# wonjune-kang/llm-speech-summarization

Hardware: AMD Instinct MI355X
Metric: generated tokens/s of end-to-end generate_audio_response steps (encode + prefill + 256-token greedy decode), HuBERT-large -> Llama-3.2-3B; audio-sec/s reported beside it, encoder stage alone and in the pipeline (higher is better)
Workload: dtype bf16

## Files before the change

### llm-speech-summarization_amd/csrc/api.hip

```cpp
#include <stdarg.h>
#include <stdlib.h>

#include <atomic>
#include <mutex>

#include "common.h"

static thread_local char g_err[512] = "";

void sl_set_error(const char* fmt, ...) {
  va_list ap;
  va_start(ap, fmt);
  vsnprintf(g_err, sizeof(g_err), fmt, ap);
  va_end(ap);
}

extern "C" const char* sl_last_error(void) { return g_err; }

extern "C" int sl_version(void) { return SL_ABI_VERSION; }

extern "C" int sl_device_arch(char* buf, int n) {
  SL_CHECK_ARG(buf != nullptr && n > 0, "sl_device_arch: bad buffer");
  int dev = 0;
  SL_HIP(hipGetDevice(&dev));
// ... 35 lines not shown
  e.stream_min_m = env_int("SL_STREAM_MIN_M", 26);
  if (e.stream_min_m < 16) e.stream_min_m = 26;
  e.disable_t256 = getenv("SL_DISABLE_T256") != nullptr;
  e.t256_min_tiles = env_int("SL_T256_MIN_TILES", 512);
  e.t256_min_k = env_int("SL_T256_MIN_K", 1024);
  e.t256_phased = env_int("SL_T256_PHASED", 1);
  e.t256_by_rounds_pad = env_int("SL_T256_BY_ROUNDS_PAD", 1);
  e.decode_tiled = env_int("SL_DECODE_TILED", 1);
  e.stream_k = env_int("SL_STREAM_K", 1);
  e.split_k = env_int("SL_SPLIT_K", 1);
  e.wgrad_tr = env_int("SL_WGRAD_TR", 1);
  e.tt_max_splits = env_int("SL_TT_MAX_SPLITS", 8);
  e.lnbwd_nw = env_int("SL_LNBWD_NW", 16);
  e.skinny_alt = env_int("SL_SKINNY_ALT", 0);
  e.prefill_share_prefix = env_int("SL_PREFILL_SHARE_PREFIX", 1);
  e.gemm_ko = env_int("SL_GEMM_KO", 0);
  { const char* sp = getenv("SL_GEMM_STAMP_PTR"); e.gemm_stamp_ptr = (sp && sp[0]) ? strtoull(sp, nullptr, 16) : 0ull; }
  const char* g = getenv("SL_DISABLE_GLDS");
  e.disable_glds = (g && g[0] == '1') ? 1 : ((g && g[0] == '2') ? 2 : 0);
  e.direct_epilogue = env_int("SL_DIRECT_EPILOGUE", 0);
  e.gemm_gm = env_int("SL_GEMM_GM", 8);
  e.attn_full_min = env_int("SL_ATTN_FULL_MIN", 32);
  e.attn_force_split = getenv("SL_ATTN_FORCE_SPLIT") != nullptr;
  { const int ks = env_int("SL_ATTN_DECODE_KS", 128); e.attn_decode_ks = (ks == 64 || ks == 65) ? ks : 128; }
  e.attn_split_merge = env_int("SL_ATTN_SPLIT_MERGE", -1);
  e.attn_generic = env_int("SL_ATTN_GENERIC", 0);
  e.attn_qt = env_int("SL_ATTN_QT", 0);
  e.norm_single_row = env_int("SL_NORM_SINGLE_ROW", 0);
  e.no_ln_fold = env_int("SL_NO_LN_FOLD", 0);
  e.no_swap_epilogue = env_int("SL_NO_SWAP_EPILOGUE", 0);
// ... 47 lines not shown
```

### llm-speech-summarization_amd/csrc/common.h

```cpp
#pragma once
#include <hip/hip_runtime.h>
#include <stdint.h>
#include <stdio.h>
#include <string.h>

#include "../../include/speechllm.h"

void sl_set_error(const char* fmt, ...);

#define SL_CHECK_ARG(cond, ...)      \
  do {                               \
    if (!(cond)) {                   \
      sl_set_error(__VA_ARGS__);     \
      return SL_ERR_ARG;             \
    }                                \
  } while (0)

#define SL_CHECK_LAUNCH(what)                                                        \
  do {                                                                               \
    hipError_t e__ = hipGetLastError();                                              \
    if (e__ != hipSuccess) {                                                         \
      sl_set_error("%s: %s", what, hipGetErrorString(e__));                          \
      return SL_ERR_LAUNCH;                                                          \
    }                                                                                \
// ... 254 lines not shown
  int direct_epilogue;
  int gemm_gm;
  int attn_full_min;
  int attn_force_split;
  int attn_decode_ks;
  int attn_split_merge;
  int attn_generic;
  int attn_qt;
  int norm_single_row;
  int no_ln_fold;
  int no_wgrad_stream;
  int gemm_log;
  int no_swap_epilogue;
  int decode_tiled;
  int prefill_share_prefix;
  int skinny_alt;
  int tt_max_splits;
  int lnbwd_nw;
  int wgrad_tr;
  int split_k;
  int stream_k;
  int gemm_ko;
  unsigned long long gemm_stamp_ptr;
  int stream_splits, stream_nwv, stream_mt;
  int stream_wide;
  int stream_wsplits;
  int stream_fixup;
  int stream_nl;
};
const SlEnv& sl_env();
// ... 22 lines not shown
```

### llm-speech-summarization_amd/csrc/gemm_stream.hip

```cpp
#include <stdlib.h>

#include <atomic>

#include "gemm_internal.h"

struct StreamX {
  float* part;
  float* part_ss;
  int splits, sps;
  int np;
  int* cnt;
  float* ss_part;
};

__device__ __forceinline__ void st_sc1_16(float* ptr, const f32x4& v) {
  asm volatile("global_store_dwordx4 %0, %1, off sc1" ::"v"(ptr), "v"(v) : "memory");
}
__device__ __forceinline__ void ld_sc1_16(f32x4& v, const float* ptr) {
  asm volatile("global_load_dwordx4 %0, %1, off sc1" : "=v"(v) : "v"(ptr) : "memory");
}
__device__ __forceinline__ void vm_drain16(f32x4 (&v)[16]) {
  asm volatile("s_waitcnt vmcnt(0)"
               : "+v"(v[0]), "+v"(v[1]), "+v"(v[2]), "+v"(v[3]), "+v"(v[4]), "+v"(v[5]), "+v"(v[6]), "+v"(v[7]), "+v"(v[8]), "+v"(v[9]), "+v"(v[10]),
                 "+v"(v[11]), "+v"(v[12]), "+v"(v[13]), "+v"(v[14]), "+v"(v[15])
// ... 478 lines not shown
      if (old == nbv - 1) s.cnt[1024 + mblock] = 0;
    }
    __builtin_amdgcn_s_barrier();
    if (!fx_last[1]) return;
    if (tid < 256) {
      const int m = m0 + tid;
      if (m < p.M) {
        float t = 0.f;
        for (int j = 0; j < nbv; ++j) t += __hip_atomic_load(&s.ss_part[(int64_t)j * p.M + m], __ATOMIC_RELAXED, __HIP_MEMORY_SCOPE_AGENT);
        sx.rstd_out[m] = rsqrtf(t / (float)p.N + sx.eps);
      }
    }
  }
}

template <typename T, int ACT, bool ROWSTAT>
__global__ __launch_bounds__(ROWSTAT ? 1024 : 256) void gemm_stream_reduce_kernel(GemmP p, SkinnyX sx, StreamX s) {
  constexpr bool PAIRS = (ACT == SL_ACT_SILU_MUL || ACT == SL_ACT_ROPE_KV);
  static_assert(!ROWSTAT || ACT == SL_ACT_NONE, "row statistics ride on the plain (+residual) epilogue");
  const int nfrag = (p.N + 15) >> 4;
  const int nunits = PAIRS ? (nfrag + 1) / 2 : nfrag;
  int q, unit, m;
  if constexpr (ROWSTAT) {
    m = blockIdx.x; q = threadIdx.x & 3; unit = threadIdx.x >> 2;
  } else {
    const int64_t idx = (int64_t)blockIdx.x * 256 + threadIdx.x;
    q = (int)(idx & 3);
    unit = (int)((idx >> 2) % nunits);
    m = (int)(idx / (4 * (int64_t)nunits));
    if (m >= p.M) return;
  }
  const bool live = unit < nunits;
  const int gf = PAIRS ? 2 * unit : unit;
  f32x4 a4 = {0.f, 0.f, 0.f, 0.f}, b4 = {0.f, 0.f, 0.f, 0.f};
  float ssum = 0.f;
  const bool stats_here = sx.fuse_rms && !sx.rstd_in;
  if (live) {
    constexpr int UN = 8;
    for (int sp0 = 0; sp0 < s.splits; sp0 += UN) {
      f32x4 va[UN], vb[UN];
#pragma unroll
      for (int u = 0; u < UN; ++u) {
        const int sp = sp0 + u < s.splits ? sp0 + u : s.splits - 1;
        const float* row = s.part + ((int64_t)sp * p.M + m) * s.np + gf * 16 + 4 * q;
        va[u] = *(const f32x4*)row;
        if constexpr (PAIRS) vb[u] = *(const f32x4*)(row + 16);
      }
#pragma unroll
      for (int u = 0; u < UN; ++u) {
        if (sp0 + u < s.splits) {
          a4 += va[u];
          if constexpr (PAIRS) b4 += vb[u];
        }
      }
    }
    if (stats_here)
      for (int sp = 0; sp < s.splits; ++sp) ssum += s.part_ss[(int64_t)sp * p.M + m];
  }
  const float rs = sx.rstd_in ? sx.rstd_in[m] : (stats_here ? rsqrtf(ssum / (float)p.K + sx.eps) : 1.0f);
  float a[4], b[4];
#pragma unroll
  for (int i = 0; i < 4; ++i) { a[i] = a4[i] * rs; b[i] = b4[i] * rs; }
  if constexpr (ROWSTAT) {
    __shared__ float wsum[17];
    float sq = 0.f;
    float kept[4] = {0.f, 0.f, 0.f, 0.f};
    if (live) {
      const T* bias = (const T*)p.bias;
#pragma unroll
      for (int i = 0; i < 4; ++i) {
        const int col = gf * 16 + 4 * q + i;
        if (col >= p.N) continue;
        float v = a[i];
        if (bias) v += to_f32(bias[col]);
        if (p.res) v += p.res_f32 ? ((const float*)p.res)[(int64_t)m * p.ldr + col] : to_f32(((const T*)p.res)[(int64_t)m * p.ldr + col]);
        if (p.out_f32) {
          ((float*)p.C)[(int64_t)m * p.ldc + col] = v;
        } else {
          const T o = from_f32<T>(v);
          ((T*)p.C)[(int64_t)m * p.ldc + col] = o;
          v = to_f32(o);
        }
        kept[i] = v;
        sq = fmaf(v, v, sq);
      }
    }
    sq = wave_sum(sq);
    if ((threadIdx.x & 63) == 0) wsum[threadIdx.x >> 6] = sq;
    __syncthreads();
    if (threadIdx.x == 0) {
      float t = 0.f;
      for (int w = 0; w < (int)(blockDim.x >> 6); ++w) t += wsum[w];
      const float rstd = rsqrtf(t / (float)p.N + sx.eps);
      sx.rstd_out[m] = rstd;
      wsum[16] = rstd;
    }
    if (sx.norm_out) {
      __syncthreads();
      const float rstd = wsum[16];
      if (live) {
        const int col0 = gf * 16 + 4 * q;
        if (col0 + 3 < p.N) {
          float o[4];
#pragma unroll
          for (int i = 0; i < 4; ++i) o[i] = to_f32(((const T*)sx.norm_gain)[col0 + i]) * to_f32(from_f32<T>(kept[i] * rstd));
          T* dst = (T*)sx.norm_out + (int64_t)m * p.N + col0;
          if constexpr (sizeof(T) == 2) *(uint2*)dst = make_uint2(pack2<T>(o[0], o[1]), pack2<T>(o[2], o[3]));
          else *(f32x4*)dst = f32x4{o[0], o[1], o[2], o[3]};
        } else {
          for (int i = 0; i < 4 && col0 + i < p.N; ++i)
            ((T*)sx.norm_out)[(int64_t)m * p.N + col0 + i] = from_f32<T>(to_f32(((const T*)sx.norm_gain)[col0 + i]) * to_f32(from_f32<T>(kept[i] * rstd)));
        }
      }
    }
  } else {
    if (live) stream_epilogue4<T, ACT>(p, sx, m, gf, 4 * q, a, b);
  }
}

struct StreamCfg { int mt, splits, nwv, d, nl; int wide, wsplits; };

static StreamCfg stream_cfg(int M, int N, int K, int kstep, bool have_ws, int dtype) {
  StreamCfg c;
  c.mt = M <= 32 ? 2 : (M <= 64 ? 4 : 8);
  const int nfrag = (N + 15) / 16;
  const int nst = K / (2 * kstep);
  c.d = 4;
  c.nl = sl_env().stream_nl ? sl_env().stream_nl : 1;
  const int sp_env = sl_env().stream_splits, nwv_env = sl_env().stream_nwv;
  if (sl_env().stream_mt && M > 64) c.mt = sl_env().stream_mt;
  const int mblocks = (M + c.mt * 16 - 1) / (c.mt * 16);
// ... 40 lines not shown
  const StreamCfg c = stream_cfg(sl_family_rows(M), N, K, dtype == SL_F32 ? 16 : 32, true, dtype);
  const int most = c.wide && c.wsplits > c.splits ? c.wsplits : c.splits;
  size_t splits = most > 1 ? (size_t)most : 0;
  return stream_ws_header(M) + splits * ((size_t)M * np + (size_t)M) * sizeof(float) + 256;
}

template <typename T, int ACT>
static int launch_stream_reduce(GemmP& p, const SkinnyX& sx, const StreamX& s, hipStream_t st) {
  if (s.splits <= 1) return 0;
  constexpr bool PAIRS = (ACT == SL_ACT_SILU_MUL || ACT == SL_ACT_ROPE_KV);
  const int nfrag = (p.N + 15) / 16;
  const int64_t nunits = PAIRS ? (nfrag + 1) / 2 : nfrag;
  const int64_t threads = (int64_t)p.M * nunits * 4;
  if constexpr (ACT == SL_ACT_NONE) {
    if (sx.rstd_out) {
      hipLaunchKernelGGL((gemm_stream_reduce_kernel<T, ACT, true>), dim3(p.M), dim3((unsigned)((nunits * 4 + 63) / 64 * 64)), 0, st, p, sx, s);
      SL_CHECK_LAUNCH("gemm_stream_reduce(rowstat)");
      return 0;
    }
  }
  hipLaunchKernelGGL((gemm_stream_reduce_kernel<T, ACT, false>), dim3((unsigned)((threads + 255) / 256)), dim3(256), 0, st, p, sx, s);
  SL_CHECK_LAUNCH("gemm_stream_reduce");
  return 0;
}

template <typename T, int MT, int ACT, int RF, int NWV, int D, int NL>
static int launch_stream_cfg(GemmP& p, const SkinnyX& sx, const StreamX& s, hipStream_t st) {
  const int nfrag = (p.N + 15) / 16;
  const int nblocks = (nfrag + NWV * RF - 1) / (NWV * RF), mblocks = (p.M + MT * 16 - 1) / (MT * 16);
  dim3 grid((nblocks + 7) / 8 * 8 * mblocks, 1, s.splits);
  if (sx.fuse_rms != 0 && sx.rstd_in == nullptr)
    hipLaunchKernelGGL((gemm_stream_kernel<T, MT, ACT, RF, NWV, D, NL, true>), grid, dim3(64 * (NWV + NL)), 0, st, p, sx, s);
  else
    hipLaunchKernelGGL((gemm_stream_kernel<T, MT, ACT, RF, NWV, D, NL, false>), grid, dim3(64 * (NWV + NL)), 0, st, p, sx, s);
  SL_CHECK_LAUNCH("gemm_stream");
  return launch_stream_reduce<T, ACT>(p, sx, s, st);
// ... 117 lines not shown
```

### llm-speech-summarization_amd/csrc/runtime.hip

```cpp
#include <vector>

#include "common.h"

int sl_attn_decode_impl(const void* q, int64_t q_stride, const void* k_cache, const void* v_cache, void* out, const int32_t* ctx_len,
                        int ctx_add, int32_t B, int32_t n_heads, int32_t n_kv, int32_t D, int32_t max_ctx, float scale, int32_t dtype,
                        hipStream_t st);
int sl_greedy_select_impl(const float* logits, int32_t B, int32_t V, const int32_t* eos_ids, int32_t n_eos, int32_t pad_id,
                          int32_t use_eos, int32_t advance_ctx, int32_t* unfinished, int32_t* ctx_len, int32_t* gen_count,
                          int32_t* finish_len, int32_t* next_ids, int32_t* out_ids, int32_t max_new, hipStream_t st, const int32_t* row_limit);
int sl_greedy_select_partial_impl(const float* amax_val, const int32_t* amax_idx, int32_t n_groups, int32_t B, const int32_t* eos_ids, int32_t n_eos,
                                  int32_t pad_id, int32_t use_eos, int32_t advance_ctx, int32_t* unfinished, int32_t* ctx_len, int32_t* gen_count,
                                  int32_t* finish_len, int32_t* next_ids, int32_t* out_ids, int32_t max_new, hipStream_t st, const int32_t* row_limit);
int sl_sample_select_impl(const float* logits, int32_t B, int32_t V, float temperature, int32_t top_k, float top_p, uint64_t seed,
                          const int32_t* eos_ids, int32_t n_eos, int32_t pad_id, int32_t use_eos, int32_t advance_ctx, int32_t* unfinished,
                          int32_t* ctx_len, int32_t* gen_count, int32_t* finish_len, int32_t* next_ids, int32_t* out_ids, int32_t max_new,
                          int32_t* choice_ws, hipStream_t st, const int32_t* row_limit, const int32_t* row_ids);

int sl_attn_decode_split_zero_counters(void* workspace, int B, int n_heads, int n_kv, int max_ctx, hipStream_t st);
int sl_attn_decode_split_impl(const void* q, int64_t q_stride, const void* k_cache, const void* v_cache, void* out, void* workspace,
                              const int32_t* ctx_len, int ctx_add, int32_t B, int32_t n_heads, int32_t n_kv, int32_t D, int32_t max_ctx,
                              float scale, int32_t dtype, hipStream_t st, int counters, int shared_prefix);
size_t sl_attn_decode_split_ws(int B, int n_heads, int n_kv, int max_ctx);
int sl_rmsnorm_rstd_impl(const void* x, void* y, const void* w, float* rstd_out, int64_t rows, int32_t cols, float eps, int32_t dtype, hipStream_t st);
int sl_gemm_impl(const sl_gemm_args* a, const sl_gemm_fused* fx, const sl_gemm_ex_args* ex, hipStream_t st);
// ... 359 lines not shown
  a.W = m->conv_w[2]; a.ldw = 3 * (int64_t)H;
  a.C = w.x; a.ldc = H; a.strideC = T * H;
  a.bias = m->conv_b[2];
  a.residual = m->pos_w; a.ldr = H; a.strideR = 0;
  a.M = (int)T; a.N = H; a.K = 3 * H; a.batch = n_utt; a.dtype = dt; a.act = SL_ACT_GELU;
  SL_TRY(sl_gemm_impl(&a, nullptr, nullptr, st));
  return encoder_tail(m, w, pl, n_utt, out, out_ld, out_row_offsets_host, last_hidden, st);
}


struct LlamaWs {
  void *h, *qkv, *att, *mid, *last, *part, *split;
  size_t split_bytes;
  float *rstd_a, *rstd_b;
  int32_t *tok_seq, *tok_pos, *cu, *cuk, *klen;
};

static size_t llama_carve(const sl_llama_model* m, int64_t n_tok, int nseq, void* base, size_t cap, LlamaWs& w) {
  const size_t sz = sl_dtype_size(m->dtype);
  const int qkv_w = (m->n_heads + 2 * m->n_kv_heads) * m->head_dim;
  Carver c(base, cap);
  w.h = c.take(n_tok * m->hidden * sz);
  w.qkv = c.take(n_tok * qkv_w * sz);
  w.att = c.take(n_tok * (int64_t)m->n_heads * m->head_dim * sz);
  w.mid = c.take(n_tok * (int64_t)m->ffn * sz);
  w.last = c.take((size_t)nseq * m->hidden * sz);
  w.part = c.take(sl_attn_decode_split_ws(nseq, m->n_heads, m->n_kv_heads, m->rope_len));
  {
    size_t sb = 0;
    const int shapes[5][2] = {{qkv_w, m->hidden}, {m->hidden, m->n_heads * m->head_dim}, {2 * m->ffn, m->hidden}, {m->hidden, m->ffn}, {m->vocab, m->hidden}};
    for (auto& sh : shapes) {
      const size_t b = sl_gemm_split_workspace_bytes(nseq, sh[0], sh[1], m->dtype);
      if (b > sb) sb = b;
    }
    w.split_bytes = sb;
    w.split = c.take(sb);
  }
  w.rstd_a = (float*)c.take((size_t)nseq * sizeof(float));
  w.rstd_b = (float*)c.take((size_t)nseq * sizeof(float));
  w.tok_seq = (int32_t*)c.take(n_tok * sizeof(int32_t));
  w.tok_pos = (int32_t*)c.take(n_tok * sizeof(int32_t));
  w.cu = (int32_t*)c.take((nseq + 2) * sizeof(int32_t));
  w.cuk = (int32_t*)c.take((nseq + 1) * sizeof(int32_t));
  w.klen = (int32_t*)c.take((nseq + 1) * sizeof(int32_t));
  return c.off + 256;
}

extern "C" size_t sl_llama_workspace_bytes(const sl_llama_model* m, int64_t n_tok, int32_t nseq) {
  LlamaWs w;
  return llama_carve(m, n_tok, nseq, nullptr, 0, w);
}

static int llama_check(const sl_llama_model* m, const sl_kv_cache* kv) {
  SL_CHECK_ARG(m && kv && m->layers && m->embed && m->lm_head && m->final_norm && m->rope_cos && m->rope_sin, "llama: null model field");
  SL_CHECK_ARG(m->head_dim == 128, "llama: head_dim %d not built (128)", m->head_dim);
  SL_CHECK_ARG(kv->k_cache && kv->v_cache && kv->slots > 0 && kv->max_ctx > 0, "llama: bad kv cache");
  SL_CHECK_ARG(kv->shared_prefix >= 0 && kv->shared_prefix <= kv->max_ctx, "llama: kv cache shared_prefix %d outside [0, max_ctx=%d]", kv->shared_prefix, kv->max_ctx);
  SL_CHECK_ARG(kv->max_ctx <= m->rope_len, "llama: max_ctx %d exceeds the rope table (%d)", kv->max_ctx, m->rope_len);
  return 0;
}

static inline size_t kv_layer_bytes(const sl_llama_model* m, const sl_kv_cache* kv) {
  return (size_t)kv->slots * m->n_kv_heads * kv->max_ctx * m->head_dim * sl_dtype_size(m->dtype);
}

__global__ __launch_bounds__(256) void gather_rows_kernel(const uint4* __restrict__ src, uint4* __restrict__ dst, const int32_t* __restrict__ map,
                                                          int64_t n_rows, int row_vec) {
  const int64_t i = (int64_t)blockIdx.x * 256 + threadIdx.x;
  if (i >= n_rows * row_vec) return;
  const int64_t r = i / row_vec;
  const int c = (int)(i - r * row_vec);
  dst[i] = src[(int64_t)map[r] * row_vec + c];
}
__global__ __launch_bounds__(64) void kv_prefix_broadcast_kernel(uint4* __restrict__ kc, uint4* __restrict__ vc, int nkv, int max_ctx, int row_vec) {
  const int pos = blockIdx.x, h = blockIdx.y, s = blockIdx.z + 1;
  uint4* c = threadIdx.x < 32 ? kc : vc;
  const int lane = threadIdx.x & 31;
  if (lane >= row_vec) return;
  const int64_t src = ((int64_t)h * max_ctx + pos) * row_vec + lane;
  c[((int64_t)s * nkv * max_ctx) * row_vec + src] = c[src];
}

__global__ __launch_bounds__(256) void weight_prefetch_kernel(const uint4* __restrict__ w, size_t n16, uint32_t* __restrict__ sink) {
  uint32_t acc = 0;
  const size_t stride = (size_t)gridDim.x * 256;
  size_t i = (size_t)blockIdx.x * 256 + threadIdx.x;
  for (; i + 7 * stride < n16; i += 8 * stride) {
// ... 38 lines not shown
  sl_gemm_fused fxl;
  if (fx_in) fxl = *fx_in; else memset(&fxl, 0, sizeof(fxl));
  fxl.split_ws = w.split; fxl.split_ws_bytes = w.split_bytes;
  fxl.rstd_in = rstd_in; fxl.rstd_out = rstd_out; fxl.rms_eps = m->rms_eps;
  fxl.norm_out = norm_out; fxl.norm_gain = norm_gain;
  const sl_gemm_fused* fx = &fxl;
  sl_gemm_args a;
  memset(&a, 0, sizeof(a));
  a.A = A; a.lda = lda; a.W = Wp; a.ldw = K; a.C = C; a.ldc = ldc; a.residual = res; a.ldr = ldc;
  a.M = M; a.N = N; a.K = K; a.batch = 1; a.dtype = m->dtype; a.act = act; a.out_f32 = out_f32; a.w_layout = SL_W_PACKED;
  return sl_gemm_impl(&a, fx, nullptr, st);
}

static int llama_layer(const sl_llama_model* m, const sl_kv_cache* kv, int l, void* x, int64_t n, LlamaWs& w, bool decode, int nseq,
                       int max_qlen, const int32_t* ctx_len_dev, hipStream_t st, bool rstd_chain = false, const float* rstd_qkv = nullptr,
                       int prefix_bcast = 0, int bcast_slots = 0, bool rstd_pass = false) {
  const sl_llama_layer& L = m->layers[l];
  const int dt = m->dtype, H = m->hidden, D = m->head_dim, nh = m->n_heads, nkv = m->n_kv_heads;
  const int qkv_w = (nh + 2 * nkv) * D;
  void* kc = bptr(kv->k_cache) + (size_t)l * kv_layer_bytes(m, kv);
  void* vc = bptr(kv->v_cache) + (size_t)l * kv_layer_bytes(m, kv);
  const float scale = 1.0f / sqrtf((float)D);
  if (decode && L.wqkv_dec && L.wo_dec && L.wgu_dec && L.wdown_dec) {
    sl_gemm_fused fx;
    memset(&fx, 0, sizeof(fx));
    fx.fuse_rms = m->dec_fused_norm; fx.rms_eps = m->rms_eps;
    fx.rope_cos = m->rope_cos; fx.rope_sin = m->rope_sin; fx.tok_pos = ctx_len_dev; fx.tok_seq = w.tok_seq;
    fx.k_cache = kc; fx.v_cache = vc; fx.n_heads = nh; fx.n_kv_heads = nkv; fx.max_ctx = kv->max_ctx;
    DecodePrefetch* pf = g_prefetch;
    const size_t esz = sl_dtype_size(dt);
    const size_t b_qkv = (size_t)qkv_w * H * esz, b_o = (size_t)H * nh * D * esz, b_gu = (size_t)2 * m->ffn * H * esz, b_down = (size_t)H * m->ffn * esz;
// ... 49 lines not shown
      const int row_vec = (int)(D * sl_dtype_size(dt) / 16);
      SL_CHECK_ARG(row_vec <= 32 && (D * sl_dtype_size(dt)) % 16 == 0, "llama: shared prefix broadcast needs K / V rows of <= 512 bytes");
      hipLaunchKernelGGL(kv_prefix_broadcast_kernel, dim3(prefix_bcast, nkv, bcast_slots - 1), dim3(64), 0, st, (uint4*)kc, (uint4*)vc, nkv, kv->max_ctx, row_vec);
      SL_CHECK_LAUNCH("kv_prefix_broadcast");
    }
    sl_attn_args a;
    memset(&a, 0, sizeof(a));
    a.q = w.qkv; a.q_row_stride = qkv_w; a.q_head_stride = D;
    a.k = kc; a.k_row_stride = D; a.k_head_stride = (int64_t)kv->max_ctx * D;
    a.v = vc; a.v_row_stride = D; a.v_head_stride = (int64_t)kv->max_ctx * D;
    a.out = w.att; a.o_row_stride = (int64_t)nh * D; a.o_head_stride = D;
    a.cu_q = w.cu; a.cu_k = w.cuk; a.klen = w.klen;
    a.nseq = nseq; a.max_qlen = max_qlen; a.n_heads = nh; a.n_kv_heads = nkv; a.head_dim = D; a.causal = 1; a.dtype = dt; a.scale = scale;
    SL_TRY(sl_attn_fwd(&a, (sl_stream)st));
  }
  SL_TRY(gemm(dt, w.att, (int64_t)nh * D, L.wo, (int64_t)nh * D, x, H, nullptr, x, H, (int)n, H, nh * D, SL_ACT_NONE, 0, st));
  SL_TRY(sl_rmsnorm(x, w.h, L.norm2, n, H, m->rms_eps, dt, (sl_stream)st));
  SL_TRY(gemm(dt, w.h, H, L.wgu, H, w.mid, m->ffn, nullptr, nullptr, 0, (int)n, 2 * m->ffn, H, SL_ACT_SILU_MUL, 0, st));
  SL_TRY(gemm(dt, w.mid, m->ffn, L.wdown, m->ffn, x, H, nullptr, x, H, (int)n, H, m->ffn, SL_ACT_NONE, 0, st));
  return 0;
}

extern "C" int sl_llama_prefill(const sl_llama_model* m, const sl_kv_cache* kv, void* x, const int32_t* cu_seqlens_host, int32_t nseq,
                                float* logits, int32_t* ctx_len_dev, void* hidden_taps, void* workspace, size_t workspace_bytes,
                                sl_stream stream) {
  SL_TRY(llama_check(m, kv));
  SL_CHECK_ARG(x && cu_seqlens_host && logits && ctx_len_dev && workspace && nseq > 0 && nseq <= kv->slots, "sl_llama_prefill: bad arguments");
  hipStream_t st = (hipStream_t)stream;
  const int64_t n_tok = cu_seqlens_host[nseq];
  const int dt = m->dtype, H = m->hidden;
  const size_t sz = sl_dtype_size(dt);
  LlamaWs w;
  const size_t need = llama_carve(m, n_tok, nseq, workspace, workspace_bytes, w);
  SL_CHECK_ARG(need <= workspace_bytes, "sl_llama_prefill: workspace %zu B < required %zu B", workspace_bytes, need);
  std::vector<int32_t> tseq(n_tok), tpos(n_tok), cuk(nseq + 1), kl(nseq + 1), ctx(nseq), cuq(nseq + 2), last_row(nseq);
  int max_q = 0;
  int P = (kv->shared_prefix > 0 && nseq > 1 && !hidden_taps && sl_env().prefill_share_prefix) ? kv->shared_prefix : 0;
  for (int s = 0; s < nseq; ++s) {
    const int len = cu_seqlens_host[s + 1] - cu_seqlens_host[s];
    SL_CHECK_ARG(len > 0 && len <= kv->max_ctx, "sl_llama_prefill: sequence %d length %d outside (0, max_ctx=%d]", s, len, kv->max_ctx);
    SL_CHECK_ARG(kv->shared_prefix <= len, "sl_llama_prefill: kv cache shared_prefix %d exceeds sequence %d (%d tokens)", kv->shared_prefix, s, len);
    if (len <= P) P = 0;
  }
  int64_t n_run = n_tok;
  int nseq_attn = nseq;
  if (P > 0) {
    std::vector<int32_t> map;
    map.reserve(n_tok);
    for (int t = 0; t < P; ++t) { map.push_back(cu_seqlens_host[0] + t); }
    cuq[0] = 0; cuq[1] = P; cuk[0] = 0; kl[0] = P;
    for (int t = 0; t < P; ++t) { tseq[t] = 0; tpos[t] = t; }
    max_q = P;
    for (int s = 0; s < nseq; ++s) {
      const int len = cu_seqlens_host[s + 1] - cu_seqlens_host[s], tail = len - P;
      const int r0 = (int)map.size();
      for (int t = 0; t < tail; ++t) { map.push_back(cu_seqlens_host[s] + P + t); tseq[r0 + t] = s; tpos[r0 + t] = P + t; }
      cuq[s + 2] = r0 + tail;
      cuk[s + 1] = s * m->n_kv_heads * kv->max_ctx;
      kl[s + 1] = len; ctx[s] = len;
      last_row[s] = r0 + tail - 1;
      if (tail > max_q) max_q = tail;
    }
    n_run = (int64_t)map.size();
    nseq_attn = nseq + 1;
    const int row_vec = (int)((size_t)H * sz / 16);
    SL_CHECK_ARG(((size_t)H * sz) % 16 == 0, "sl_llama_prefill: hidden rows must be a multiple of 16 bytes");
    SL_HIP(hipMemcpyAsync(w.tok_pos, map.data(), n_run * sizeof(int32_t), hipMemcpyHostToDevice, st));
    hipLaunchKernelGGL(gather_rows_kernel, dim3((unsigned)((n_run * row_vec + 255) / 256)), dim3(256), 0, st, (const uint4*)x, (uint4*)w.mid, w.tok_pos, n_run, row_vec);
    SL_CHECK_LAUNCH("gather_rows");
    SL_HIP(hipMemcpyAsync(x, w.mid, (size_t)n_run * H * sz, hipMemcpyDeviceToDevice, st));
    SL_HIP(hipStreamSynchronize(st));
  } else {
    for (int s = 0; s < nseq; ++s) {
      const int len = cu_seqlens_host[s + 1] - cu_seqlens_host[s];
      for (int t = 0; t < len; ++t) { tseq[cu_seqlens_host[s] + t] = s; tpos[cu_seqlens_host[s] + t] = t; }
      cuk[s] = s * m->n_kv_heads * kv->max_ctx;
      kl[s] = len; ctx[s] = len;
      cuq[s] = cu_seqlens_host[s];
      last_row[s] = cu_seqlens_host[s + 1] - 1;
      if (len > max_q) max_q = len;
    }
    cuq[nseq] = cu_seqlens_host[nseq];
  }
  SL_HIP(hipMemcpyAsync(w.tok_seq, tseq.data(), n_run * sizeof(int32_t), hipMemcpyHostToDevice, st));
  SL_HIP(hipMemcpyAsync(w.tok_pos, tpos.data(), n_run * sizeof(int32_t), hipMemcpyHostToDevice, st));
  SL_HIP(hipMemcpyAsync(w.cu, cuq.data(), (nseq_attn + 1) * sizeof(int32_t), hipMemcpyHostToDevice, st));
  SL_HIP(hipMemcpyAsync(w.cuk, cuk.data(), nseq_attn * sizeof(int32_t), hipMemcpyHostToDevice, st));
  SL_HIP(hipMemcpyAsync(w.klen, kl.data(), nseq_attn * sizeof(int32_t), hipMemcpyHostToDevice, st));
  SL_HIP(hipMemcpyAsync(ctx_len_dev, ctx.data(), nseq * sizeof(int32_t), hipMemcpyHostToDevice, st));
  SL_HIP(hipStreamSynchronize(st));
  for (int l = 0; l < m->n_layers; ++l) {
    if (hidden_taps) SL_HIP(hipMemcpyAsync(bptr(hidden_taps) + (size_t)l * n_tok * H * sz, x, n_tok * H * sz, hipMemcpyDeviceToDevice, st));
    SL_TRY(llama_layer(m, kv, l, x, n_run, w, false, nseq_attn, max_q, nullptr, st, false, nullptr, P, nseq));
  }
  if (hidden_taps) {
    SL_TRY(sl_rmsnorm(x, bptr(hidden_taps) + (size_t)m->n_layers * n_tok * H * sz, m->final_norm, n_tok, H, m->rms_eps, dt, stream));
  }
  for (int s = 0; s < nseq; ++s)
    SL_HIP(hipMemcpyAsync(bptr(w.last) + (size_t)s * H * sz, bptr(x) + (size_t)last_row[s] * H * sz, H * sz, hipMemcpyDeviceToDevice, st));
  SL_TRY(sl_rmsnorm(w.last, w.last, m->final_norm, nseq, H, m->rms_eps, dt, stream));
  SL_TRY(gemm(dt, w.last, H, m->lm_head, H, logits, m->vocab, nullptr, nullptr, 0, nseq, m->vocab, H, SL_ACT_NONE, 1, st));
  return 0;
}

constexpr int SL_FUSED_ARGMAX_MIN_B = 256;

static bool decode_fuses_argmax(const sl_llama_model* m, int B) { B = sl_family_rows(B); return B > 64 && !(m->lm_head_dec && B < SL_FUSED_ARGMAX_MIN_B); }

static int decode_step(const sl_llama_model* m, const sl_kv_cache* kv, const int32_t* next_ids, const int32_t* ctx_len, int B, float* logits,
                       void* x, LlamaWs& w, hipStream_t st, bool fused_top1 = false) {
  const int dt = m->dtype, H = m->hidden;
  SL_TRY(sl_embed_gather(m->embed, next_ids, x, B, H, dt, (sl_stream)st));
  bool chain = m->dec_fused_norm && m->lm_head_dec && H / 16 * 4 <= 1024 && H % 16 == 0 &&
               sl_gemm_split_count(B, H, m->n_heads * m->head_dim, dt) > 1 && sl_gemm_split_count(B, H, m->ffn, dt) > 1 && w.split != nullptr;
// ... 419 lines not shown
```

Before: 66810.

## Prune final prefill layer to last rows and rework rowstat split-k reduce

In prefill, the last Llama layer now runs its output projection, norm and MLP only on each sequence's last token, gathered by a device-side row map, because only those rows feed the LM head. The per-sequence last-row copies become one gather kernel. Separately, the split-K stream reduce with row statistics is moved into its own kernel: 256 threads per row, multiple column chunks per thread, vectorized residual, gain and store, and a fast path for aligned bf16 residual-only cases. This trims prefill FLOPs and reduce-kernel overhead, at the cost of more kernel variants. The pruned path reuses workspace buffers (qkv, last, mid), so it must not overlap live data.

```diff
diff --git a/llm-speech-summarization_amd/csrc/api.hip b/llm-speech-summarization_amd/csrc/api.hip
--- a/llm-speech-summarization_amd/csrc/api.hip
+++ b/llm-speech-summarization_amd/csrc/api.hip
@@ -73,6 +73,7 @@
   e.lnbwd_nw = env_int("SL_LNBWD_NW", 16);
   e.skinny_alt = env_int("SL_SKINNY_ALT", 0);
   e.prefill_share_prefix = env_int("SL_PREFILL_SHARE_PREFIX", 1);
+  e.prefill_prune_last = env_int("SL_PREFILL_PRUNE_LAST", 1);
   e.gemm_ko = env_int("SL_GEMM_KO", 0);
   { const char* sp = getenv("SL_GEMM_STAMP_PTR"); e.gemm_stamp_ptr = (sp && sp[0]) ? strtoull(sp, nullptr, 16) : 0ull; }
   const char* g = getenv("SL_DISABLE_GLDS");
diff --git a/llm-speech-summarization_amd/csrc/common.h b/llm-speech-summarization_amd/csrc/common.h
--- a/llm-speech-summarization_amd/csrc/common.h
+++ b/llm-speech-summarization_amd/csrc/common.h
@@ -292,6 +292,7 @@
   int no_swap_epilogue;
   int decode_tiled;
   int prefill_share_prefix;
+  int prefill_prune_last;
   int skinny_alt;
   int tt_max_splits;
   int lnbwd_nw;
diff --git a/llm-speech-summarization_amd/csrc/gemm_stream.hip b/llm-speech-summarization_amd/csrc/gemm_stream.hip
--- a/llm-speech-summarization_amd/csrc/gemm_stream.hip
+++ b/llm-speech-summarization_amd/csrc/gemm_stream.hip
@@ -1,3 +1,4 @@
+#include <type_traits>
 #include <stdlib.h>
 
 #include <atomic>
@@ -516,107 +517,259 @@
   }
 }
 
-template <typename T, int ACT, bool ROWSTAT>
-__global__ __launch_bounds__(ROWSTAT ? 1024 : 256) void gemm_stream_reduce_kernel(GemmP p, SkinnyX sx, StreamX s) {
+template <int UN, int NCH, bool PAIRS>
+__device__ __forceinline__ void reduce_add_splits(const float* rec, int64_t split_stride, int sp0, const uint32_t (&voff)[NCH], f32x4 (&a4)[NCH],
+                                                  f32x4 (&b4)[NCH]) {
+  f32x4 va[NCH][UN], vb[NCH][UN];
+#pragma unroll
+  for (int u = 0; u < UN; ++u) {
+    const float* row = rec + (int64_t)(sp0 + u) * split_stride;
+#pragma unroll
+    for (int j = 0; j < NCH; ++j) {
+      va[j][u] = *(const f32x4*)(row + voff[j]);
+      if constexpr (PAIRS) vb[j][u] = *(const f32x4*)(row + voff[j] + 16);
+    }
+  }
+#pragma unroll
+  for (int u = 0; u < UN; ++u)
+#pragma unroll
+    for (int j = 0; j < NCH; ++j) {
+      a4[j] += va[j][u];
+      if constexpr (PAIRS) b4[j] += vb[j][u];
+    }
+}
+template <int UNMAX, int NCH, bool PAIRS>
+__device__ __forceinline__ void reduce_sum_splits(const float* rec, int64_t split_stride, int splits, const uint32_t (&voff)[NCH], f32x4 (&a4)[NCH],
+                                                  f32x4 (&b4)[NCH]) {
+  int sp0 = 0;
+  for (; sp0 + UNMAX <= splits; sp0 += UNMAX) reduce_add_splits<UNMAX, NCH, PAIRS>(rec, split_stride, sp0, voff, a4, b4);
+  if constexpr (UNMAX > 4) {
+    if (splits - sp0 >= 4) { reduce_add_splits<4, NCH, PAIRS>(rec, split_stride, sp0, voff, a4, b4); sp0 += 4; }
+  }
+  if constexpr (UNMAX > 2) {
+    if (splits - sp0 >= 2) { reduce_add_splits<2, NCH, PAIRS>(rec, split_stride, sp0, voff, a4, b4); sp0 += 2; }
+  }
+  if constexpr (UNMAX > 1) {
+    if (splits - sp0 >= 1) reduce_add_splits<1, NCH, PAIRS>(rec, split_stride, sp0, voff, a4, b4);
+  }
+}
+
+template <typename T, int ACT>
+__global__ __launch_bounds__(256) void gemm_stream_reduce_kernel(GemmP p, SkinnyX sx, StreamX s) {
   constexpr bool PAIRS = (ACT == SL_ACT_SILU_MUL || ACT == SL_ACT_ROPE_KV);
-  static_assert(!ROWSTAT || ACT == SL_ACT_NONE, "row statistics ride on the plain (+residual) epilogue");
   const int nfrag = (p.N + 15) >> 4;
   const int nunits = PAIRS ? (nfrag + 1) / 2 : nfrag;
-  int q, unit, m;
-  if constexpr (ROWSTAT) {
-    m = blockIdx.x; q = threadIdx.x & 3; unit = threadIdx.x >> 2;
-  } else {
-    const int64_t idx = (int64_t)blockIdx.x * 256 + threadIdx.x;
-    q = (int)(idx & 3);
-    unit = (int)((idx >> 2) % nunits);
-    m = (int)(idx / (4 * (int64_t)nunits));
-    if (m >= p.M) return;
-  }
-  const bool live = unit < nunits;
+  const int64_t idx = (int64_t)blockIdx.x * 256 + threadIdx.x;
+  const int q = (int)(idx & 3);
+  const int unit = (int)((idx >> 2) % nunits);
+  const int m = (int)(idx / (4 * (int64_t)nunits));
+  if (m >= p.M) return;
   const int gf = PAIRS ? 2 * unit : unit;
-  f32x4 a4 = {0.f, 0.f, 0.f, 0.f}, b4 = {0.f, 0.f, 0.f, 0.f};
+  f32x4 a4[1] = {{0.f, 0.f, 0.f, 0.f}}, b4[1] = {{0.f, 0.f, 0.f, 0.f}};
+  const uint32_t voff[1] = {0u};
+  reduce_sum_splits<8, 1, PAIRS>(s.part + (int64_t)m * s.np + gf * 16 + 4 * q, (int64_t)p.M * s.np, s.splits, voff, a4, b4);
   float ssum = 0.f;
   const bool stats_here = sx.fuse_rms && !sx.rstd_in;
-  if (live) {
-    constexpr int UN = 8;
-    for (int sp0 = 0; sp0 < s.splits; sp0 += UN) {
-      f32x4 va[UN], vb[UN];
-#pragma unroll
-      for (int u = 0; u < UN; ++u) {
-        const int sp = sp0 + u < s.splits ? sp0 + u : s.splits - 1;
-        const float* row = s.part + ((int64_t)sp * p.M + m) * s.np + gf * 16 + 4 * q;
-        va[u] = *(const f32x4*)row;
-        if constexpr (PAIRS) vb[u] = *(const f32x4*)(row + 16);
-      }
-#pragma unroll
-      for (int u = 0; u < UN; ++u) {
-        if (sp0 + u < s.splits) {
-          a4 += va[u];
-          if constexpr (PAIRS) b4 += vb[u];
-        }
-      }
-    }
-    if (stats_here)
-      for (int sp = 0; sp < s.splits; ++sp) ssum += s.part_ss[(int64_t)sp * p.M + m];
-  }
+  if (stats_here)
+    for (int sp = 0; sp < s.splits; ++sp) ssum += s.part_ss[(int64_t)sp * p.M + m];
   const float rs = sx.rstd_in ? sx.rstd_in[m] : (stats_here ? rsqrtf(ssum / (float)p.K + sx.eps) : 1.0f);
   float a[4], b[4];
 #pragma unroll
-  for (int i = 0; i < 4; ++i) { a[i] = a4[i] * rs; b[i] = b4[i] * rs; }
-  if constexpr (ROWSTAT) {
-    __shared__ float wsum[17];
+  for (int i = 0; i < 4; ++i) { a[i] = a4[0][i] * rs; b[i] = b4[0][i] * rs; }
+  stream_epilogue4<T, ACT>(p, sx, m, gf, 4 * q, a, b);
+}
+
+template <typename T>
+__device__ __forceinline__ float norm_round(float x, float rstd) {
+  float y = x * rstd;
+  asm volatile("" : "+v"(y));
+  return to_f32(from_f32<T>(y));
+}
+
+template <typename T, int NCH, bool FAST>
+__global__ __launch_bounds__(256) void gemm_stream_reduce_rowstat_kernel(GemmP p, SkinnyX sx, StreamX s) {
+  __shared__ float wsum[16];
+  const int nfrag = (p.N + 15) >> 4;
+  const int ngroups = (4 * nfrag + 63) >> 6;
+  const int m = blockIdx.x, tid = threadIdx.x;
+  uint32_t col0[NCH], voff[NCH];
+  bool live[NCH];
+#pragma unroll
+  for (int j = 0; j < NCH; ++j) {
+    col0[j] = 4u * (uint32_t)(j * 256 + tid);
+    live[j] = col0[j] < (FAST ? (uint32_t)p.N : 16u * (uint32_t)nfrag);
+    voff[j] = live[j] ? col0[j] : 0u;
+  }
+  float kept[NCH][4];
+  if constexpr (FAST) {
+    typedef typename std::conditional<sizeof(T) == 2, uint2, f32x4>::type Piece;
+    Piece rr[NCH];
+#pragma unroll
+    for (int j = 0; j < NCH; ++j) rr[j] = *(const Piece*)((const T*)p.res + (int64_t)m * p.ldr + voff[j]);
+    f32x4 a4[NCH], b4[NCH];
+#pragma unroll
+    for (int j = 0; j < NCH; ++j) a4[j] = b4[j] = f32x4{0.f, 0.f, 0.f, 0.f};
+    reduce_sum_splits<(NCH >= 3 ? 2 : 4), NCH, false>(s.part + (int64_t)m * s.np, (int64_t)p.M * s.np, s.splits, voff, a4, b4);
+#pragma unroll
+    for (int j = 0; j < NCH; ++j) {
+      float v[4];
+      if constexpr (sizeof(T) == 2) {
+        const f32x2_t lo = unpack2<T>(rr[j].x), hi = unpack2<T>(rr[j].y);
+        v[0] = a4[j][0] + lo.x; v[1] = a4[j][1] + lo.y; v[2] = a4[j][2] + hi.x; v[3] = a4[j][3] + hi.y;
+        const uint32_t plo = pack2<T>(v[0], v[1]), phi = pack2<T>(v[2], v[3]);
+        if (live[j]) *(uint2*)((T*)p.C + (int64_t)m * p.ldc + col0[j]) = make_uint2(plo, phi);
+        const f32x2_t f01 = unpack2<T>(plo), f23 = unpack2<T>(phi);
+        v[0] = f01.x; v[1] = f01.y; v[2] = f23.x; v[3] = f23.y;
+      } else {
+#pragma unroll
+        for (int i = 0; i < 4; ++i) v[i] = a4[j][i] + rr[j][i];
+        if (live[j]) *(f32x4*)((float*)p.C + (int64_t)m * p.ldc + col0[j]) = f32x4{v[0], v[1], v[2], v[3]};
+      }
+      float sq = 0.f;
+#pragma unroll
+      for (int i = 0; i < 4; ++i) { kept[j][i] = v[i]; sq = fmaf(v[i], v[i], sq); }
+      sq = wave_sum(live[j] ? sq : 0.f);
+      if ((tid & 63) == 0) wsum[j * 4 + (tid >> 6)] = sq;
+    }
+  } else {
+  const bool res16 = !p.res_f32 && sizeof(T) == 2;
+  const bool vec_res = p.res && !(p.ldr & 3) && !((uintptr_t)p.res & (res16 ? 7 : 15));
+  const bool vec_c = !(p.ldc & 3) && !((uintptr_t)p.C & ((p.out_f32 || sizeof(T) == 4) ? 15 : 7));
+  float r[NCH][4];
+#pragma unroll
+  for (int j = 0; j < NCH; ++j) {
+#pragma unroll
+    for (int i = 0; i < 4; ++i) r[j][i] = 0.f;
+    if (!p.res || !live[j]) continue;
+    const int64_t off = (int64_t)m * p.ldr + col0[j];
+    if (vec_res && col0[j] + 3 < (uint32_t)p.N) {
+      if (res16) {
+        if constexpr (sizeof(T) == 2) {
+          const uint2 w = *(const uint2*)((const T*)p.res + off);
+          const f32x2_t lo = unpack2<T>(w.x), hi = unpack2<T>(w.y);
+          r[j][0] = lo.x; r[j][1] = lo.y; r[j][2] = hi.x; r[j][3] = hi.y;
+        }
+      } else {
+        const f32x4 w = *(const f32x4*)((const float*)p.res + off);
+#pragma unroll
+        for (int i = 0; i < 4; ++i) r[j][i] = w[i];
+      }
+    } else {
+      for (int i = 0; i < 4 && col0[j] + i < (uint32_t)p.N; ++i)
+        r[j][i] = p.res_f32 ? ((const float*)p.res)[off + i] : to_f32(((const T*)p.res)[off + i]);
+    }
+  }
+  f32x4 a4[NCH], b4[NCH];
+#pragma unroll
+  for (int j = 0; j < NCH; ++j) a4[j] = b4[j] = f32x4{0.f, 0.f, 0.f, 0.f};
+  reduce_sum_splits<(NCH >= 3 ? 2 : 4), NCH, false>(s.part + (int64_t)m * s.np, (int64_t)p.M * s.np, s.splits, voff, a4, b4);
+  float ssum = 0.f;
+  const bool stats_here = sx.fuse_rms && !sx.rstd_in;
+  if (stats_here)
+    for (int sp = 0; sp < s.splits; ++sp) ssum += s.part_ss[(int64_t)sp * p.M + m];
+  const float rs = sx.rstd_in ? sx.rstd_in[m] : (stats_here ? rsqrtf(ssum / (float)p.K + sx.eps) : 1.0f);
+  const T* bias = (const T*)p.bias;
+#pragma unroll
+  for (int j = 0; j < NCH; ++j) {
     float sq = 0.f;
-    float kept[4] = {0.f, 0.f, 0.f, 0.f};
-    if (live) {
-      const T* bias = (const T*)p.bias;
+#pragma unroll
+    for (int i = 0; i < 4; ++i) kept[j][i] = 0.f;
+    if (live[j]) {
+      const int64_t off = (int64_t)m * p.ldc + col0[j];
+      const bool whole = col0[j] + 3 < (uint32_t)p.N;
+      float v[4];
 #pragma unroll
       for (int i = 0; i < 4; ++i) {
-        const int col = gf * 16 + 4 * q + i;
-        if (col >= p.N) continue;
-        float v = a[i];
-        if (bias) v += to_f32(bias[col]);
-        if (p.res) v += p.res_f32 ? ((const float*)p.res)[(int64_t)m * p.ldr + col] : to_f32(((const T*)p.res)[(int64_t)m * p.ldr + col]);
+        v[i] = a4[j][i] * rs;
+        if (bias && col0[j] + i < (uint32_t)p.N) v[i] += to_f32(bias[col0[j] + i]);
+        if (p.res) v[i] += r[j][i];
+      }
+      if (whole && vec_c) {
         if (p.out_f32) {
-          ((float*)p.C)[(int64_t)m * p.ldc + col] = v;
+          *(f32x4*)((float*)p.C + off) = f32x4{v[0], v[1], v[2], v[3]};
+        } else if constexpr (sizeof(T) == 2) {
+          const uint32_t lo = pack2<T>(v[0], v[1]), hi = pack2<T>(v[2], v[3]);
+          *(uint2*)((T*)p.C + off) = make_uint2(lo, hi);
+          const f32x2_t f01 = unpack2<T>(lo), f23 = unpack2<T>(hi);
+          v[0] = f01.x; v[1] = f01.y; v[2] = f23.x; v[3] = f23.y;
         } else {
-          const T o = from_f32<T>(v);
-          ((T*)p.C)[(int64_t)m * p.ldc + col] = o;
-          v = to_f32(o);
-        }
-        kept[i] = v;
-        sq = fmaf(v, v, sq);
+          *(f32x4*)((float*)p.C + off) = f32x4{v[0], v[1], v[2], v[3]};
+        }
+#pragma unroll
+        for (int i = 0; i < 4; ++i) { kept[j][i] = v[i]; sq = fmaf(v[i], v[i], sq); }
+      } else {
+#pragma unroll
+        for (int i = 0; i < 4; ++i) {
+          if (col0[j] + i >= (uint32_t)p.N) continue;
+          if (p.out_f32) {
+            ((float*)p.C)[off + i] = v[i];
+          } else {
+            const T o = from_f32<T>(v[i]);
+            ((T*)p.C)[off + i] = o;
+            v[i] = to_f32(o);
+          }
+          kept[j][i] = v[i];
+          sq = fmaf(v[i], v[i], sq);
+        }
       }
     }
     sq = wave_sum(sq);
-    if ((threadIdx.x & 63) == 0) wsum[threadIdx.x >> 6] = sq;
-    __syncthreads();
-    if (threadIdx.x == 0) {
-      float t = 0.f;
-      for (int w = 0; w < (int)(blockDim.x >> 6); ++w) t += wsum[w];
-      const float rstd = rsqrtf(t / (float)p.N + sx.eps);
-      sx.rstd_out[m] = rstd;
-      wsum[16] = rstd;
-    }
+    if ((tid & 63) == 0) wsum[j * 4 + (tid >> 6)] = sq;
+  }
+  }
+  typedef typename std::conditional<sizeof(T) == 2, uint2, f32x4>::type GainPiece;
+  GainPiece gg[NCH];
+  if constexpr (FAST) {
     if (sx.norm_out) {
-      __syncthreads();
-      const float rstd = wsum[16];
-      if (live) {
-        const int col0 = gf * 16 + 4 * q;
-        if (col0 + 3 < p.N) {
-          float o[4];
-#pragma unroll
-          for (int i = 0; i < 4; ++i) o[i] = to_f32(((const T*)sx.norm_gain)[col0 + i]) * to_f32(from_f32<T>(kept[i] * rstd));
-          T* dst = (T*)sx.norm_out + (int64_t)m * p.N + col0;
-          if constexpr (sizeof(T) == 2) *(uint2*)dst = make_uint2(pack2<T>(o[0], o[1]), pack2<T>(o[2], o[3]));
-          else *(f32x4*)dst = f32x4{o[0], o[1], o[2], o[3]};
+#pragma unroll
+      for (int j = 0; j < NCH; ++j) gg[j] = *(const GainPiece*)((const T*)sx.norm_gain + voff[j]);
+    }
+  }
+  __syncthreads();
+  float t = 0.f;
+  for (int g = 0; g < ngroups; ++g) t += wsum[g];
+  const float rstd = rsqrtf(t / (float)p.N + sx.eps);
+  if (tid == 0) sx.rstd_out[m] = rstd;
+  if (sx.norm_out) {
+    const bool vec_g = FAST || !((uintptr_t)sx.norm_gain & (sizeof(T) == 2 ? 7 : 15));
+    const bool vec_n = FAST || (!(p.N & 3) && !((uintptr_t)sx.norm_out & (sizeof(T) == 2 ? 7 : 15)));
+#pragma unroll
+    for (int j = 0; j < NCH; ++j) {
+      if (!live[j]) continue;
+      const T* gain = (const T*)sx.norm_gain + col0[j];
+      T* dst = (T*)sx.norm_out + (int64_t)m * p.N + col0[j];
+      if (FAST || (col0[j] + 3 < (uint32_t)p.N && vec_n)) {
+        float g4[4], o[4];
+        if constexpr (FAST) {
+          if constexpr (sizeof(T) == 2) {
+            const f32x2_t lo = unpack2<T>(gg[j].x), hi = unpack2<T>(gg[j].y);
+            g4[0] = lo.x; g4[1] = lo.y; g4[2] = hi.x; g4[3] = hi.y;
+          } else {
+#pragma unroll
+            for (int i = 0; i < 4; ++i) g4[i] = gg[j][i];
+          }
+        } else if constexpr (sizeof(T) == 2) {
+          if (vec_g) {
+            const uint2 w = *(const uint2*)gain;
+            const f32x2_t lo = unpack2<T>(w.x), hi = unpack2<T>(w.y);
+            g4[0] = lo.x; g4[1] = lo.y; g4[2] = hi.x; g4[3] = hi.y;
+          } else {
+#pragma unroll
+            for (int i = 0; i < 4; ++i) g4[i] = to_f32(gain[i]);
+          }
         } else {
-          for (int i = 0; i < 4 && col0 + i < p.N; ++i)
-            ((T*)sx.norm_out)[(int64_t)m * p.N + col0 + i] = from_f32<T>(to_f32(((const T*)sx.norm_gain)[col0 + i]) * to_f32(from_f32<T>(kept[i] * rstd)));
-        }
-      }
-    }
-  } else {
-    if (live) stream_epilogue4<T, ACT>(p, sx, m, gf, 4 * q, a, b);
+#pragma unroll
+          for (int i = 0; i < 4; ++i) g4[i] = to_f32(gain[i]);
+        }
+#pragma unroll
+        for (int i = 0; i < 4; ++i) o[i] = g4[i] * norm_round<T>(kept[j][i], rstd);
+        if constexpr (sizeof(T) == 2) *(uint2*)dst = make_uint2(pack2<T>(o[0], o[1]), pack2<T>(o[2], o[3]));
+        else *(f32x4*)dst = f32x4{o[0], o[1], o[2], o[3]};
+      } else {
+        for (int i = 0; i < 4 && col0[j] + i < (uint32_t)p.N; ++i)
+          dst[i] = from_f32<T>(to_f32(gain[i]) * norm_round<T>(kept[j][i], rstd));
+      }
+    }
   }
 }
 
@@ -687,12 +840,23 @@
   const int64_t threads = (int64_t)p.M * nunits * 4;
   if constexpr (ACT == SL_ACT_NONE) {
     if (sx.rstd_out) {
-      hipLaunchKernelGGL((gemm_stream_reduce_kernel<T, ACT, true>), dim3(p.M), dim3((unsigned)((nunits * 4 + 63) / 64 * 64)), 0, st, p, sx, s);
+      const uintptr_t al = sizeof(T) == 2 ? 7 : 15;
+      const bool fast = !p.bias && p.res && !p.res_f32 && !p.out_f32 && !sx.fuse_rms && !sx.rstd_in && !(p.N & 3) && !(p.ldc & 3) && !(p.ldr & 3) &&
+                        !((uintptr_t)p.C & al) && !((uintptr_t)p.res & al) && (!sx.norm_out || (!((uintptr_t)sx.norm_out & al) && !((uintptr_t)sx.norm_gain & al)));
+      const int nch = (nfrag * 4 + 255) / 256;
+#define SL_ROWSTAT_LAUNCH(NCH_)                                                                                                              \
+  if (fast) hipLaunchKernelGGL((gemm_stream_reduce_rowstat_kernel<T, NCH_, true>), dim3(p.M), dim3(256), 0, st, p, sx, s);                   \
+  else hipLaunchKernelGGL((gemm_stream_reduce_rowstat_kernel<T, NCH_, false>), dim3(p.M), dim3(256), 0, st, p, sx, s)
+      if (nch <= 1) { SL_ROWSTAT_LAUNCH(1); }
+      else if (nch == 2) { SL_ROWSTAT_LAUNCH(2); }
+      else if (nch == 3) { SL_ROWSTAT_LAUNCH(3); }
+      else { SL_ROWSTAT_LAUNCH(4); }
+#undef SL_ROWSTAT_LAUNCH
       SL_CHECK_LAUNCH("gemm_stream_reduce(rowstat)");
       return 0;
     }
   }
-  hipLaunchKernelGGL((gemm_stream_reduce_kernel<T, ACT, false>), dim3((unsigned)((threads + 255) / 256)), dim3(256), 0, st, p, sx, s);
+  hipLaunchKernelGGL((gemm_stream_reduce_kernel<T, ACT>), dim3((unsigned)((threads + 255) / 256)), dim3(256), 0, st, p, sx, s);
   SL_CHECK_LAUNCH("gemm_stream_reduce");
   return 0;
 }
diff --git a/llm-speech-summarization_amd/csrc/runtime.hip b/llm-speech-summarization_amd/csrc/runtime.hip
--- a/llm-speech-summarization_amd/csrc/runtime.hip
+++ b/llm-speech-summarization_amd/csrc/runtime.hip
@@ -397,6 +397,7 @@
   size_t split_bytes;
   float *rstd_a, *rstd_b;
   int32_t *tok_seq, *tok_pos, *cu, *cuk, *klen;
+  int32_t* last_row;
 };
 
 static size_t llama_carve(const sl_llama_model* m, int64_t n_tok, int nseq, void* base, size_t cap, LlamaWs& w) {
@@ -426,6 +427,7 @@
   w.cu = (int32_t*)c.take((nseq + 2) * sizeof(int32_t));
   w.cuk = (int32_t*)c.take((nseq + 1) * sizeof(int32_t));
   w.klen = (int32_t*)c.take((nseq + 1) * sizeof(int32_t));
+  w.last_row = (int32_t*)c.take((size_t)nseq * sizeof(int32_t));
   return c.off + 256;
 }
 
@@ -454,6 +456,12 @@
   const int64_t r = i / row_vec;
   const int c = (int)(i - r * row_vec);
   dst[i] = src[(int64_t)map[r] * row_vec + c];
+}
+static int gather_rows(const void* src, void* dst, const int32_t* map, int64_t n_rows, size_t row_bytes, hipStream_t st) {
+  const int row_vec = (int)(row_bytes / 16);
+  hipLaunchKernelGGL(gather_rows_kernel, dim3((unsigned)((n_rows * row_vec + 255) / 256)), dim3(256), 0, st, (const uint4*)src, (uint4*)dst, map, n_rows, row_vec);
+  SL_CHECK_LAUNCH("gather_rows");
+  return 0;
 }
 __global__ __launch_bounds__(64) void kv_prefix_broadcast_kernel(uint4* __restrict__ kc, uint4* __restrict__ vc, int nkv, int max_ctx, int row_vec) {
   const int pos = blockIdx.x, h = blockIdx.y, s = blockIdx.z + 1;
@@ -522,7 +530,7 @@
 
 static int llama_layer(const sl_llama_model* m, const sl_kv_cache* kv, int l, void* x, int64_t n, LlamaWs& w, bool decode, int nseq,
                        int max_qlen, const int32_t* ctx_len_dev, hipStream_t st, bool rstd_chain = false, const float* rstd_qkv = nullptr,
-                       int prefix_bcast = 0, int bcast_slots = 0, bool rstd_pass = false) {
+                       int prefix_bcast = 0, int bcast_slots = 0, bool rstd_pass = false, const int32_t* tail_rows = nullptr, int n_tail = 0) {
   const sl_llama_layer& L = m->layers[l];
   const int dt = m->dtype, H = m->hidden, D = m->head_dim, nh = m->n_heads, nkv = m->n_kv_heads;
   const int qkv_w = (nh + 2 * nkv) * D;
@@ -602,6 +610,18 @@
     a.nseq = nseq; a.max_qlen = max_qlen; a.n_heads = nh; a.n_kv_heads = nkv; a.head_dim = D; a.causal = 1; a.dtype = dt; a.scale = scale;
     SL_TRY(sl_attn_fwd(&a, (sl_stream)st));
   }
+  if (tail_rows && !decode) {
+    const size_t esz = sl_dtype_size(dt);
+    void* att_t = w.qkv;
+    SL_TRY(gather_rows(w.att, att_t, tail_rows, n_tail, (size_t)nh * D * esz, st));
+    SL_TRY(gather_rows(x, w.last, tail_rows, n_tail, (size_t)H * esz, st));
+    SlFamilyPin pin((int)n);
+    SL_TRY(gemm(dt, att_t, (int64_t)nh * D, L.wo, (int64_t)nh * D, w.last, H, nullptr, w.last, H, n_tail, H, nh * D, SL_ACT_NONE, 0, st));
+    SL_TRY(sl_rmsnorm(w.last, w.h, L.norm2, n_tail, H, m->rms_eps, dt, (sl_stream)st));
+    SL_TRY(gemm(dt, w.h, H, L.wgu, H, w.mid, m->ffn, nullptr, nullptr, 0, n_tail, 2 * m->ffn, H, SL_ACT_SILU_MUL, 0, st));
+    SL_TRY(gemm(dt, w.mid, m->ffn, L.wdown, m->ffn, w.last, H, nullptr, w.last, H, n_tail, H, m->ffn, SL_ACT_NONE, 0, st));
+    return 0;
+  }
   SL_TRY(gemm(dt, w.att, (int64_t)nh * D, L.wo, (int64_t)nh * D, x, H, nullptr, x, H, (int)n, H, nh * D, SL_ACT_NONE, 0, st));
   SL_TRY(sl_rmsnorm(x, w.h, L.norm2, n, H, m->rms_eps, dt, (sl_stream)st));
   SL_TRY(gemm(dt, w.h, H, L.wgu, H, w.mid, m->ffn, nullptr, nullptr, 0, (int)n, 2 * m->ffn, H, SL_ACT_SILU_MUL, 0, st));
@@ -621,6 +641,7 @@
   LlamaWs w;
   const size_t need = llama_carve(m, n_tok, nseq, workspace, workspace_bytes, w);
   SL_CHECK_ARG(need <= workspace_bytes, "sl_llama_prefill: workspace %zu B < required %zu B", workspace_bytes, need);
+  SL_CHECK_ARG(((size_t)H * sz) % 16 == 0, "sl_llama_prefill: hidden rows must be a multiple of 16 bytes");
   std::vector<int32_t> tseq(n_tok), tpos(n_tok), cuk(nseq + 1), kl(nseq + 1), ctx(nseq), cuq(nseq + 2), last_row(nseq);
   int max_q = 0;
   int P = (kv->shared_prefix > 0 && nseq > 1 && !hidden_taps && sl_env().prefill_share_prefix) ? kv->shared_prefix : 0;
@@ -651,11 +672,8 @@
     }
     n_run = (int64_t)map.size();
     nseq_attn = nseq + 1;
-    const int row_vec = (int)((size_t)H * sz / 16);
-    SL_CHECK_ARG(((size_t)H * sz) % 16 == 0, "sl_llama_prefill: hidden rows must be a multiple of 16 bytes");
     SL_HIP(hipMemcpyAsync(w.tok_pos, map.data(), n_run * sizeof(int32_t), hipMemcpyHostToDevice, st));
-    hipLaunchKernelGGL(gather_rows_kernel, dim3((unsigned)((n_run * row_vec + 255) / 256)), dim3(256), 0, st, (const uint4*)x, (uint4*)w.mid, w.tok_pos, n_run, row_vec);
-    SL_CHECK_LAUNCH("gather_rows");
+    SL_TRY(gather_rows(x, w.mid, w.tok_pos, n_run, (size_t)H * sz, st));
     SL_HIP(hipMemcpyAsync(x, w.mid, (size_t)n_run * H * sz, hipMemcpyDeviceToDevice, st));
     SL_HIP(hipStreamSynchronize(st));
   } else {
@@ -676,16 +694,18 @@
   SL_HIP(hipMemcpyAsync(w.cuk, cuk.data(), nseq_attn * sizeof(int32_t), hipMemcpyHostToDevice, st));
   SL_HIP(hipMemcpyAsync(w.klen, kl.data(), nseq_attn * sizeof(int32_t), hipMemcpyHostToDevice, st));
   SL_HIP(hipMemcpyAsync(ctx_len_dev, ctx.data(), nseq * sizeof(int32_t), hipMemcpyHostToDevice, st));
+  SL_HIP(hipMemcpyAsync(w.last_row, last_row.data(), nseq * sizeof(int32_t), hipMemcpyHostToDevice, st));
   SL_HIP(hipStreamSynchronize(st));
+  const bool prune = !hidden_taps && m->n_layers > 0 && sl_env().prefill_prune_last != 0;
   for (int l = 0; l < m->n_layers; ++l) {
     if (hidden_taps) SL_HIP(hipMemcpyAsync(bptr(hidden_taps) + (size_t)l * n_tok * H * sz, x, n_tok * H * sz, hipMemcpyDeviceToDevice, st));
-    SL_TRY(llama_layer(m, kv, l, x, n_run, w, false, nseq_attn, max_q, nullptr, st, false, nullptr, P, nseq));
+    const bool tail = prune && l == m->n_layers - 1;
+    SL_TRY(llama_layer(m, kv, l, x, n_run, w, false, nseq_attn, max_q, nullptr, st, false, nullptr, P, nseq, false, tail ? w.last_row : nullptr, nseq));
   }
   if (hidden_taps) {
     SL_TRY(sl_rmsnorm(x, bptr(hidden_taps) + (size_t)m->n_layers * n_tok * H * sz, m->final_norm, n_tok, H, m->rms_eps, dt, stream));
   }
-  for (int s = 0; s < nseq; ++s)
-    SL_HIP(hipMemcpyAsync(bptr(w.last) + (size_t)s * H * sz, bptr(x) + (size_t)last_row[s] * H * sz, H * sz, hipMemcpyDeviceToDevice, st));
+  if (!prune) SL_TRY(gather_rows(x, w.last, w.last_row, nseq, (size_t)H * sz, st));
   SL_TRY(sl_rmsnorm(w.last, w.last, m->final_norm, nseq, H, m->rms_eps, dt, stream));
   SL_TRY(gemm(dt, w.last, H, m->lm_head, H, logits, m->vocab, nullptr, nullptr, 0, nseq, m->vocab, H, SL_ACT_NONE, 1, st));
   return 0;
```

Result: faster. 68220, median of 6 (+2.1%).
